# ajbrock/Neural-Photo-Editor

Hardware: NVIDIA H100
Metric: 64x64 images/sec IAN encode->decode @ batch 256 (higher is better)
Workload: dtype f32 (3-pass bf16 split on wgmma, fp32 accumulate)

## Files before the change

### neural-photo-editor_b200/csrc/tapgemm_tc.cu

```cuda
#include <cuda.h>

#include <cstdio>
#include <cstring>
#include <vector>

#include "tapgemm.h"
#include "tc_ptx.cuh"

namespace ian {

struct TcMaps {
  CUtensorMap a[4];
  CUtensorMap b;
  CUtensorMap a1[4];
  CUtensorMap b1;
  CUtensorMap o[2];
  const __nv_bfloat16* o_out;
  long long o_plane;
  int Wt, Ht, Nt, BN;
  mutable int sk_choice;
};

namespace {

using namespace tc;

constexpr int BM = 128;
constexpr int BK = 64;

constexpr int kEpiWarps = 8;
constexpr int kThreadsCta = 32 * kEpiWarps + 32;

template <int BN, int PASSES> struct TcCfg {
  static constexpr int kPlanes = PASSES == 3 ? 2 : 1;
  static constexpr int kATileBytes = BM * BK * 2 * kPlanes;
  static constexpr int kBTileBytes = BN * BK * 2 * kPlanes;
  static constexpr int kStageBytes = kATileBytes + kBTileBytes;
  static constexpr int kRound = (PASSES == 3 && BN > 32) ? 32 : BN;
  static constexpr int kRounds = BN / kRound;
  static constexpr int kLd = kRound + 8;
  static constexpr bool kTmaEpi = PASSES == 3 && BN == 128;
  static constexpr int kOutPlaneBytes = BM * kRound * 2;
  static constexpr int kOutRoundBytes = 2 * kOutPlaneBytes;
  static constexpr int kStagingBytes = kTmaEpi && 2 * kOutRoundBytes > BM * kLd * 4 ? 2 * kOutRoundBytes : BM * kLd * 4;
  static constexpr int kStageSmem = kTmaEpi ? 1024 : kEpiWarps * 1024;
  static constexpr int kStagesFit = (232448 - 1024 - 256 - kStagingBytes - kStageSmem) / kStageBytes;
  static constexpr int kStages = kStagesFit > 6 ? 6 : kStagesFit;
  static constexpr int kSmemBytes = kStages * kStageBytes + 1024  + 256  + kStageSmem + kStagingBytes;
  static_assert(kStages >= 2 && kSmemBytes <= 232448, "tapgemm_tc: shared memory budget");
};
static_assert(TcCfg<128, 3>::kStages == 3 && TcCfg<128, 3>::kSmemBytes == 231680, "tapgemm_tc: three float32-mode stages");
static_assert(TcCfg<128, 3>::kRound == 32 && TcCfg<128, 3>::kOutRoundBytes == 16384, "tapgemm_tc: 32-column TMA-store rounds");

struct WorkItem {
  int phase, ks, co0, it0, it1;
  int n0, p0, q0, mtile;
  int sk_role, sk_last;
};

template <int CH, int PASSES>
__device__ __forceinline__ void store_split(__nv_bfloat16* dst, long long plane, const float (&v)[CH]) {
  __align__(16) __nv_bfloat162 hi[CH / 2], lo[CH / 2];
#pragma unroll
  for (int j = 0; j < CH / 2; ++j) {
    hi[j] = __floats2bfloat162_rn(v[2 * j], v[2 * j + 1]);
    if (PASSES == 3) {
      const float2 hf = __bfloat1622float2(hi[j]);
      lo[j] = __floats2bfloat162_rn(v[2 * j] - hf.x, v[2 * j + 1] - hf.y);
    }
  }
  static_assert(CH % 16 == 0, "an epilogue chunk is a whole number of 32-byte sectors per plane");
  const uint4* h4 = reinterpret_cast<const uint4*>(hi);
  const uint4* l4 = reinterpret_cast<const uint4*>(lo);
#pragma unroll
  for (int j = 0; j < CH / 16; ++j) {
    tc::st_global_256(dst + 16 * j, h4[2 * j], h4[2 * j + 1]);
    if (PASSES == 3) tc::st_global_256(dst + plane + 16 * j, l4[2 * j], l4[2 * j + 1]);
  }
}

template <int BN>
__device__ __forceinline__ WorkItem decode_work(const TapGemm& g, const TcMaps& maps, int w) {
  WorkItem wi;
  const int tiles_q = g.Wg / maps.Wt, tiles_p = g.Hg / maps.Ht;
  const int tiles_m = tiles_q * tiles_p * ((g.n_img + maps.Nt - 1) / maps.Nt);
  const int tiles_n = g.Cout / BN;
  const int per_phase = tiles_m * tiles_n * g.ksplit;
  wi.phase = w / per_phase;
  int r = w % per_phase;
  int mt = r % tiles_m; r /= tiles_m;
  const int nt = r % tiles_n; r /= tiles_n;
  wi.ks = r;
  wi.mtile = mt;
  const int qb = mt % tiles_q; mt /= tiles_q;
  const int pb = mt % tiles_p; mt /= tiles_p;
  wi.n0 = mt * maps.Nt; wi.p0 = pb * maps.Ht; wi.q0 = qb * maps.Wt;
  wi.co0 = nt * BN;
  const int total_it = g.phase[wi.phase].ntaps * (g.Cin / BK);
  wi.it0 = (int)((long long)total_it * wi.ks / g.ksplit);
  wi.it1 = (int)((long long)total_it * (wi.ks + 1) / g.ksplit);
  return wi;
}

template <int BN, bool SK>
struct WorkIter {
  int w, total, stride;
  int T, G, cur, end, iters[kMaxPhases], tiles_per_phase, tiles_m, tiles_q, tiles_p;
  __device__ __forceinline__ int boundary(int c) const { return (int)((long long)T * c / G); }
  __device__ __forceinline__ int owner(int gi) const {
    int c = (int)((long long)gi * G / T);
    while (c + 1 < G && boundary(c + 1) <= gi) ++c;
    while (c > 0 && boundary(c) > gi) --c;
    return c;
  }
  __device__ __forceinline__ void init(const TapGemm& g, const TcMaps& maps, int total_work) {
    if (!SK) { w = blockIdx.x; total = total_work; stride = gridDim.x; return; }
    T = total_work; G = gridDim.x;
    tiles_q = g.Wg / maps.Wt; tiles_p = g.Hg / maps.Ht;
    tiles_m = tiles_q * tiles_p * ((g.n_img + maps.Nt - 1) / maps.Nt);
    tiles_per_phase = tiles_m * (g.Cout / BN);
    for (int p = 0; p < kMaxPhases; ++p) iters[p] = p < g.nphase ? g.phase[p].ntaps * (g.Cin / BK) : 0;
    cur = boundary(blockIdx.x); end = boundary(blockIdx.x + 1);
  }
  __device__ __forceinline__ bool next(const TapGemm& g, const TcMaps& maps, WorkItem& wi) {
    if (!SK) {
      if (w >= total) return false;
      wi = decode_work<BN>(g, maps, w);
      wi.sk_role = 0; wi.sk_last = 0;
      w += stride;
      return true;
    }
    if (cur >= end) return false;
    int gi = cur, ph = 0, phase_start = 0;
    while (ph + 1 < g.nphase && gi >= phase_start + tiles_per_phase * iters[ph]) { phase_start += tiles_per_phase * iters[ph]; ++ph; }
    const int ip = iters[ph];
    const int tile = (gi - phase_start) / ip, it = (gi - phase_start) % ip;
    int len = ip - it;
    if (len > end - gi) len = end - gi;
    wi.phase = ph; wi.ks = 0; wi.it0 = it; wi.it1 = it + len;
    int mt = tile % tiles_m;
    const int nt = tile / tiles_m;
    wi.mtile = mt;
    const int qb = mt % tiles_q; mt /= tiles_q;
    const int pb = mt % tiles_p; mt /= tiles_p;
    wi.n0 = mt * maps.Nt; wi.p0 = pb * maps.Ht; wi.q0 = qb * maps.Wt; wi.co0 = nt * BN;
    wi.sk_role = it > 0 ? 1 : (len < ip ? 2 : 0);
    wi.sk_last = wi.sk_role == 2 ? owner(phase_start + tile * ip + ip - 1) : 0;
    cur = gi + len;
    return true;
  }
};

template <int BN, int PASSES, bool SK>
__global__ void __launch_bounds__(kThreadsCta, 1)
tapgemm_tc_kernel(const __grid_constant__ TapGemm g, const __grid_constant__ TcMaps maps, const int total_work) {
  using Cfg = TcCfg<BN, PASSES>;
  constexpr int kATileBytes = Cfg::kATileBytes;
  constexpr int S = Cfg::kStages;
  extern __shared__ uint8_t smem_raw[];
  const uint32_t smem_base = (smem_u32(smem_raw) + 1023u) & ~1023u;
  const uint32_t stg_base = smem_base + S * Cfg::kStageBytes;
  const uint32_t bar_base = stg_base + Cfg::kStagingBytes;
  auto full_bar = [&](int s) { return bar_base + 8u * s; };
  auto empty_bar = [&](int s) { return bar_base + 8u * (S + s); };
  const uint32_t stage_smem = bar_base + 256u;
  uint8_t* smem_al = smem_raw + (smem_base - smem_u32(smem_raw));
  float* stage_ptr = reinterpret_cast<float*>(smem_al + (stage_smem - smem_base));
  float* acc_tile = reinterpret_cast<float*>(smem_al + (stg_base - smem_base));

  const int warp = threadIdx.x >> 5, lane = threadIdx.x & 31;

  if (threadIdx.x == 0) {
    pdl_trigger();
    for (int s = 0; s < S; ++s) {
      mbar_init(full_bar(s), 1);
      mbar_init(empty_bar(s), 2);
    }
    asm volatile("fence.mbarrier_init.release.cluster;" ::: "memory");
  }
  __syncthreads();
  pdl_wait();

  if (warp == kEpiWarps) {
    uint32_t i = 0;
    WorkIter<BN, SK> iter;
    iter.init(g, maps, total_work);
    WorkItem wi;
    while (iter.next(g, maps, wi)) {
      const Phase ph = g.phase[wi.phase];
      int t = wi.it0 % ph.ntaps, c0 = wi.it0 / ph.ntaps * BK;
      for (int it = wi.it0; it < wi.it1; ++it, ++i) {
        const int s = i % S;
        const uint32_t par = (i / S) & 1u;
        const Tap tap = g.taps[ph.tap_begin + t];
        mbar_wait(empty_bar(s), par ^ 1u);
        const uint32_t sa = smem_base + s * Cfg::kStageBytes;
        if (elect_one_sync()) {
          mbar_expect_tx(full_bar(s), Cfg::kStageBytes);
          tma_load_5d(PASSES == 3 ? &maps.a[tap.view] : &maps.a1[tap.view], full_bar(s), sa, c0, wi.q0 + tap.dw,
                      wi.p0 + tap.dh, wi.n0, 0);
          tma_load_3d(PASSES == 3 ? &maps.b : &maps.b1, full_bar(s), sa + kATileBytes, c0, tap.wtile * g.Cout + wi.co0, 0);
        }
        __syncwarp();
        if (++t == ph.ntaps) { t = 0; c0 += BK; }
      }
    }
    return;
  }

  constexpr int R = BN / 2;
  constexpr int RW = Cfg::kRound;
  constexpr int TC = RW >= 32 ? RW / 2 : RW;
  constexpr int CH = TC >= 32 ? 32 : 16;
  constexpr int kThreadCols = Cfg::kRounds * TC;
  const int wg = warp >> 2, wtid = threadIdx.x & 127;
  const int ew = warp;
  const int lg = warp & 3;
  const int half = ew >> 2;
  const bool has_cols = RW >= 32 || half == 0;
  float* my_stage = stage_ptr + (Cfg::kTmaEpi ? 0 : ew * 256);
  const float act_a = g.act == ACT_LRELU ? 0.6f : g.act == ACT_RELU ? 0.5f : 1.f;
  const float act_b = g.act == ACT_LRELU ? 0.4f : g.act == ACT_RELU ? 0.5f : 0.f;
  const int ml = lg * 32 + lane;
  const int wl0 = ml % maps.Wt;
  const int hl0 = (ml / maps.Wt) % maps.Ht;
  const int nl0 = ml / (maps.Wt * maps.Ht);
  uint32_t i = 0;
  WorkIter<BN, SK> iter;
  iter.init(g, maps, total_work);
  WorkItem wi;
  while (iter.next(g, maps, wi)) {
    const Phase ph = g.phase[wi.phase];
    if (wi.it1 <= wi.it0) continue;
    if (g.scale_pix_stride == 0) {
      if constexpr (Cfg::kTmaEpi) {
        asm volatile("bar.sync 1, 256;" ::: "memory");
        for (int c = threadIdx.x; c < BN; c += 32 * kEpiWarps) {
          my_stage[c] = g.scale ? __ldg(g.scale + wi.co0 + c) : 1.f;
          my_stage[128 + c] = g.shift ? __ldg(g.shift + wi.co0 + c) : 0.f;
        }
      } else if (has_cols) {
        __syncwarp();
        for (int c = lane; c < BN; c += 32) {
          my_stage[c] = g.scale ? __ldg(g.scale + wi.co0 + c) : 1.f;
          my_stage[128 + c] = g.shift ? __ldg(g.shift + wi.co0 + c) : 0.f;
        }
        __syncwarp();
      }
    }
    float acc_m[R], acc_c[PASSES == 3 ? R : 1];
#pragma unroll
    for (int j = 0; j < R; ++j) acc_m[j] = 0.f;
#pragma unroll
    for (int j = 0; j < (PASSES == 3 ? R : 1); ++j) acc_c[j] = 0.f;
    wgmma_fence_regs(acc_m);
    if (PASSES == 3) wgmma_fence_regs(acc_c);
    for (int it = wi.it0; it < wi.it1; ++it, ++i) {
      const int s = i % S;
      mbar_wait(full_bar(s), (i / S) & 1u);
      const uint32_t sa = smem_base + s * Cfg::kStageBytes;
      const uint64_t a_hi = make_sw128_desc(sa + wg * 64 * 128), a_lo = make_sw128_desc(sa + BM * BK * 2 + wg * 64 * 128);
      const uint64_t b_hi = make_sw128_desc(sa + kATileBytes), b_lo = make_sw128_desc(sa + kATileBytes + BN * BK * 2);
      const uint32_t first = (it == wi.it0) ? 0u : 1u;
      wgmma_fence();
#pragma unroll
      for (int k = 0; k < BK / 16; ++k) {
        const uint64_t ko = (uint64_t)(k * 2);
        const uint32_t acc = k > 0 ? 1u : first;
        wgmma_bf16<BN>(acc_m, a_hi + ko, b_hi + ko, acc);
        if constexpr (PASSES == 3) {
          wgmma_bf16<BN>(acc_c, a_lo + ko, b_hi + ko, acc);
          wgmma_bf16<BN>(acc_c, a_hi + ko, b_lo + ko, 1u);
        }
      }
      wgmma_commit();
      wgmma_wait<1>();
      if (it > wi.it0 && wtid == 0) mbar_arrive(empty_bar((i - 1) % S));
    }
    wgmma_wait<0>();
    wgmma_fence_regs(acc_m);
    if (PASSES == 3) wgmma_fence_regs(acc_c);
    if (wtid == 0) mbar_arrive(empty_bar((i - 1) % S));
    if constexpr (PASSES == 3) {
#pragma unroll
      for (int j = 0; j < R; ++j) acc_m[j] += acc_c[j];
    }
    if constexpr (Cfg::kTmaEpi) {
      if (g.epi_tma && wi.sk_role == 0) {
#pragma unroll
        for (int r = 0; r < Cfg::kRounds; ++r) {
          const uint32_t buf = stg_base + (uint32_t)(r & 1) * Cfg::kOutRoundBytes;
          if (threadIdx.x == 0) bulk_wait_group_read1();
          asm volatile("bar.sync 1, 256;" ::: "memory");
#pragma unroll
          for (int j = 0; j < RW / 2; j += 2) {
            const float2 a = make_float2(acc_m[r * RW / 2 + j], acc_m[r * RW / 2 + j + 1]);
            const int row = wg * 64 + frag_row(wtid, j);
            const int c = frag_col(wtid, j);
            const float2 sc = *reinterpret_cast<const float2*>(my_stage + r * RW + c);
            const float2 sf = *reinterpret_cast<const float2*>(my_stage + 128 + r * RW + c);
            float v0 = fmaf(a.x, sc.x, sf.x), v1 = fmaf(a.y, sc.y, sf.y);
            if (g.act == ACT_ELU) {
              v0 = v0 > 0.f ? v0 : expm1f(v0);
              v1 = v1 > 0.f ? v1 : expm1f(v1);
            } else if (g.act != ACT_NONE) {
              v0 = fmaf(act_b, fabsf(v0), act_a * v0);
              v1 = fmaf(act_b, fabsf(v1), act_a * v1);
            }
            const __nv_bfloat162 hi = __floats2bfloat162_rn(v0, v1);
            const float2 hf = __bfloat1622float2(hi);
            const __nv_bfloat162 lo = __floats2bfloat162_rn(v0 - hf.x, v1 - hf.y);
            const uint32_t off = (uint32_t)row * 64u + ((((uint32_t)c >> 3) ^ (((uint32_t)row >> 1) & 3u)) << 4) + ((uint32_t)c & 7u) * 2u;
            asm volatile("st.shared.b32 [%0], %1;" ::"r"(buf + off), "r"(*reinterpret_cast<const uint32_t*>(&hi)) : "memory");
            asm volatile("st.shared.b32 [%0], %1;" ::"r"(buf + Cfg::kOutPlaneBytes + off), "r"(*reinterpret_cast<const uint32_t*>(&lo))
                         : "memory");
          }
          fence_proxy_async_smem();
          asm volatile("bar.sync 1, 256;" ::: "memory");
          if (threadIdx.x == 0) {
            const int c4 = wi.n0 * g.Hg + wi.p0;
            tma_store_5d(&maps.o[0], buf, wi.co0 + r * RW, ph.ow0, wi.q0, ph.oh0, c4);
            tma_store_5d(&maps.o[1], buf + Cfg::kOutPlaneBytes, wi.co0 + r * RW, ph.ow0, wi.q0, ph.oh0, c4);
            bulk_commit_group();
          }
        }
        continue;
      }
      if (threadIdx.x == 0) bulk_wait_group_read0();
    }
    if (SK && wi.sk_role == 2 && has_cols) {
      for (int k = (int)blockIdx.x + 1 + lane; k <= wi.sk_last; k += 32) {
        if (iter.boundary(k) == iter.boundary(k + 1)) continue;
        const int* fl = g.sk_flags + k * kEpiWarps + ew;
        const long long t0 = clock64();
        int fv;
        do {
          asm volatile("ld.acquire.gpu.global.s32 %0, [%1];" : "=r"(fv) : "l"(fl) : "memory");
          if (clock64() - t0 > 4000000000LL) __trap();
        } while (fv != g.sk_epoch);
      }
      __syncwarp();
    }
    int nl = nl0, hl = hl0, wl = wl0;
    if constexpr (SK && Cfg::kTmaEpi) {
      uint32_t tid;
      asm volatile("mov.u32 %0, %%tid.x;" : "=r"(tid));
      const int row = (int)((tid >> 5) & 3u) * 32 + (int)(tid & 31u);
      wl = row % maps.Wt;
      hl = (row / maps.Wt) % maps.Ht;
      nl = row / (maps.Wt * maps.Ht);
    }
    const int n = wi.n0 + nl, p = wi.p0 + hl, q = wi.q0 + wl;
    const bool valid = n < g.n_img;
    const int oh = p * g.osh + ph.oh0, ow = q * g.osw + ph.ow0;
    const long long pix = (long long)(n * g.Hout + oh) * g.Wout + ow;
#pragma unroll 1
    for (int r = 0; r < Cfg::kRounds; ++r) {
      asm volatile("bar.sync 1, 256;" ::: "memory");
#pragma unroll
      for (int j = 0; j < RW / 2; j += 2) {
        float2 v = make_float2(acc_m[j], acc_m[j + 1]);
#pragma unroll
        for (int rr = 1; rr < Cfg::kRounds; ++rr)
          if (rr == r) v = make_float2(acc_m[rr * RW / 2 + j], acc_m[rr * RW / 2 + j + 1]);
        *reinterpret_cast<float2*>(acc_tile + (wg * 64 + frag_row(wtid, j)) * Cfg::kLd + frag_col(wtid, j)) = v;
      }
      asm volatile("bar.sync 1, 256;" ::: "memory");
      if (!has_cols) continue;
#pragma unroll 1
      for (int cc = 0; cc < TC; cc += CH) {
        const int cb = r * RW + half * TC + cc;
        const int co = wi.co0 + cb;
        const int cs = r * TC + cc;
        float v[CH];
        const float* srow = acc_tile + ml * Cfg::kLd + half * TC + cc;
#pragma unroll
        for (int j = 0; j < CH / 4; ++j) {
          const float4 t4 = *reinterpret_cast<const float4*>(srow + 4 * j);
          v[4 * j] = t4.x; v[4 * j + 1] = t4.y; v[4 * j + 2] = t4.z; v[4 * j + 3] = t4.w;
        }
        if (SK && wi.sk_role == 1) {
          float4* wp = reinterpret_cast<float4*>(g.sk_ws + (((long long)blockIdx.x * kEpiWarps + ew) * 32 + lane) * kThreadCols + cs);
#pragma unroll
          for (int j = 0; j < CH / 4; ++j) __stcg(wp + j, make_float4(v[4 * j], v[4 * j + 1], v[4 * j + 2], v[4 * j + 3]));
          continue;
        }
        if (SK && wi.sk_role == 2) {
          for (int k = (int)blockIdx.x + 1; k <= wi.sk_last; ++k) {
            if (iter.boundary(k) == iter.boundary(k + 1)) continue;
            const float4* rp = reinterpret_cast<const float4*>(g.sk_ws + (((long long)k * kEpiWarps + ew) * 32 + lane) * kThreadCols + cs);
#pragma unroll
            for (int j = 0; j < CH / 4; ++j) {
              const float4 a = __ldcg(rp + j);
              v[4 * j] += a.x; v[4 * j + 1] += a.y; v[4 * j + 2] += a.z; v[4 * j + 3] += a.w;
            }
          }
        }
        if (g.ksplit > 1) {
          if (valid) {
            float4* wsp = reinterpret_cast<float4*>(g.ws + (long long)wi.ks * g.ws_slab + pix * g.Cout + co);
#pragma unroll
            for (int j = 0; j < CH / 4; ++j) __stcg(wsp + j, make_float4(v[4 * j], v[4 * j + 1], v[4 * j + 2], v[4 * j + 3]));
          }
          continue;
        }
        if (valid) {
          const long long off = pix * g.Cout + co;
          if (g.out_raw) store_split<CH, PASSES>(g.out_raw + off, g.out_raw_plane, v);
          if (g.res && !g.res_after) {
            const uint4* rh = reinterpret_cast<const uint4*>(g.res + off);
            const uint4* rl = reinterpret_cast<const uint4*>(g.res + g.res_plane + off);
#pragma unroll
            for (int j8 = 0; j8 < CH / 8; ++j8) {
              const uint4 h4 = __ldg(rh + j8);
              const __nv_bfloat16* hb = reinterpret_cast<const __nv_bfloat16*>(&h4);
              if (PASSES == 3) {
                const uint4 l4 = __ldg(rl + j8);
                const __nv_bfloat16* lb = reinterpret_cast<const __nv_bfloat16*>(&l4);
#pragma unroll
                for (int j = 0; j < 8; ++j) v[j8 * 8 + j] += __bfloat162float(hb[j]) + __bfloat162float(lb[j]);
              } else {
#pragma unroll
                for (int j = 0; j < 8; ++j) v[j8 * 8 + j] += __bfloat162float(hb[j]);
              }
            }
          }
          if (g.act == ACT_MASK) {
            const int si = co + (oh * g.Wout + ow) * g.scale_pix_stride;
            const uint4* mk = reinterpret_cast<const uint4*>(g.mask + off);
#pragma unroll
            for (int j8 = 0; j8 < CH / 8; ++j8) {
              const uint4 m4 = __ldg(mk + j8);
              const __nv_bfloat16* mb = reinterpret_cast<const __nv_bfloat16*>(&m4);
#pragma unroll
              for (int j = 0; j < 8; ++j) {
                const float sc = g.scale_pix_stride ? __ldg(g.scale + si + j8 * 8 + j) : my_stage[cb + j8 * 8 + j];
                v[j8 * 8 + j] = v[j8 * 8 + j] * sc * (__bfloat162float(mb[j]) > 0.f ? 1.f : g.mask_slope);
              }
            }
            if (g.res && g.res_after) {
              const uint4* rh = reinterpret_cast<const uint4*>(g.res + off);
              const uint4* rl = reinterpret_cast<const uint4*>(g.res + g.res_plane + off);
#pragma unroll
              for (int j8 = 0; j8 < CH / 8; ++j8) {
                const uint4 h4 = __ldg(rh + j8);
                const __nv_bfloat16* hb = reinterpret_cast<const __nv_bfloat16*>(&h4);
                if (PASSES == 3) {
                  const uint4 l4 = __ldg(rl + j8);
                  const __nv_bfloat16* lb = reinterpret_cast<const __nv_bfloat16*>(&l4);
#pragma unroll
                  for (int j = 0; j < 8; ++j) v[j8 * 8 + j] += __bfloat162float(hb[j]) + __bfloat162float(lb[j]);
                } else {
#pragma unroll
                  for (int j = 0; j < 8; ++j) v[j8 * 8 + j] += __bfloat162float(hb[j]);
                }
              }
            }
          } else {
#pragma unroll
            for (int j4 = 0; j4 < CH / 4; ++j4) {
              const float4 sc = *reinterpret_cast<const float4*>(my_stage + cb + 4 * j4);
              const float4 sf = *reinterpret_cast<const float4*>(my_stage + 128 + cb + 4 * j4);
              v[4 * j4 + 0] = fmaf(v[4 * j4 + 0], sc.x, sf.x);
              v[4 * j4 + 1] = fmaf(v[4 * j4 + 1], sc.y, sf.y);
              v[4 * j4 + 2] = fmaf(v[4 * j4 + 2], sc.z, sf.z);
              v[4 * j4 + 3] = fmaf(v[4 * j4 + 3], sc.w, sf.w);
            }
            if (g.act == ACT_ELU) {
#pragma unroll
              for (int j = 0; j < CH; ++j) v[j] = v[j] > 0.f ? v[j] : expm1f(v[j]);
            } else if (g.act != ACT_NONE) {
#pragma unroll
              for (int j = 0; j < CH; ++j) v[j] = fmaf(act_b, fabsf(v[j]), act_a * v[j]);
            }
          }
          if (g.out) store_split<CH, PASSES>(g.out + off, g.out_plane, v);
          if (g.out_f32_t) {
            const long long tbase = ((long long)wi.mtile * g.cout_real + co) * BM + ml;
            if (g.out_t_bf16) {
              __nv_bfloat16* ot = reinterpret_cast<__nv_bfloat16*>(g.out_f32_t) + tbase;
#pragma unroll
              for (int j = 0; j < CH; ++j)
                if (co + j < g.cout_real) ot[j * BM] = __float2bfloat16_rn(v[j]);
            } else {
              float* ot = g.out_f32_t + tbase;
#pragma unroll
              for (int j = 0; j < CH; ++j)
                if (co + j < g.cout_real) ot[j * BM] = v[j];
            }
          }
          if (g.out_f32) {
            float4* of = reinterpret_cast<float4*>(g.out_f32 + off);
#pragma unroll
            for (int j = 0; j < CH / 4; ++j) of[j] = make_float4(v[4 * j], v[4 * j + 1], v[4 * j + 2], v[4 * j + 3]);
          }
        }
      }
    }
    if (SK && wi.sk_role == 1 && has_cols) {
      __threadfence();
      __syncwarp();
      if (lane == 0) {
        int* fl = g.sk_flags + (int)blockIdx.x * kEpiWarps + ew;
        asm volatile("st.release.gpu.global.s32 [%0], %1;" ::"l"(fl), "r"(g.sk_epoch) : "memory");
      }
    }
  }
  if constexpr (Cfg::kTmaEpi) {
    if (threadIdx.x == 0) bulk_wait_group0();
  }
}

}

TcMaps* tc_build_maps(const TapGemm& g, char* err, int errlen) {
  tc::EncodeTiledFn enc = tc::get_encode_fn();
  if (!enc) { snprintf(err, errlen, "cuTensorMapEncodeTiled entry point not available"); return nullptr; }
  if (g.Cin % 64 || (g.Cout % 128 && g.Cout != 16)) { snprintf(err, errlen, "tc path needs Cin%%64==0 and Cout%%128==0 or Cout==16 (got %d,%d)", g.Cin, g.Cout); return nullptr; }
  TcMaps* m = new TcMaps();
  memset(m, 0, sizeof(*m));
  tile_shape(g.Hg, g.Wg, m->Wt, m->Ht, m->Nt);
  m->sk_choice = -1;
  m->BN = (g.Cout % 128 == 0) ? 128 : 16;
  if (g.Wg % m->Wt || g.Hg % m->Ht || m->Wt * m->Ht * m->Nt != BM) {
    snprintf(err, errlen, "M grid %dx%d does not tile into 128-row boxes", g.Hg, g.Wg);
    delete m; return nullptr;
  }
  bool used[4] = {false, false, false, false};
  int max_tile = 0;
  for (int p = 0; p < g.nphase; ++p)
    for (int t = 0; t < g.phase[p].ntaps; ++t) {
      const Tap& tp = g.taps[g.phase[p].tap_begin + t];
      used[tp.view] = true;
      if (tp.wtile > max_tile) max_tile = tp.wtile;
    }
  for (int v = 0; v < 4; ++v) {
    if (!used[v]) continue;
    const int vh = v >> 1, vw = v & 1;
    const cuuint64_t Hv = (g.Hin - vh + g.sh - 1) / g.sh, Wv = (g.Win - vw + g.sw - 1) / g.sw;
    cuuint64_t dims[5] = {(cuuint64_t)g.Cin, Wv, Hv, (cuuint64_t)g.n_img, 2};
    cuuint64_t strides[4] = {(cuuint64_t)g.sw * g.Cin * 2, (cuuint64_t)g.sh * g.Win * g.Cin * 2,
                             (cuuint64_t)g.Hin * g.Win * g.Cin * 2, (cuuint64_t)g.a_plane * 2};
    cuuint32_t box[5] = {BK, (cuuint32_t)m->Wt, (cuuint32_t)m->Ht, (cuuint32_t)m->Nt, 2};
    cuuint32_t estr[5] = {1, 1, 1, 1, 1};
    void* base = (void*)(g.a + ((long long)vh * g.Win + vw) * g.Cin);
    CUresult r = enc(&m->a[v], CU_TENSOR_MAP_DATA_TYPE_BFLOAT16, 5, base, dims, strides, box, estr,
                     CU_TENSOR_MAP_INTERLEAVE_NONE, CU_TENSOR_MAP_SWIZZLE_128B, CU_TENSOR_MAP_L2_PROMOTION_L2_256B,
                     CU_TENSOR_MAP_FLOAT_OOB_FILL_NONE);
    if (r != CUDA_SUCCESS) { snprintf(err, errlen, "cuTensorMapEncodeTiled(A view %d) failed: %d", v, (int)r); delete m; return nullptr; }
    box[4] = 1;
    r = enc(&m->a1[v], CU_TENSOR_MAP_DATA_TYPE_BFLOAT16, 5, base, dims, strides, box, estr, CU_TENSOR_MAP_INTERLEAVE_NONE,
            CU_TENSOR_MAP_SWIZZLE_128B, CU_TENSOR_MAP_L2_PROMOTION_L2_256B, CU_TENSOR_MAP_FLOAT_OOB_FILL_NONE);
    if (r != CUDA_SUCCESS) { snprintf(err, errlen, "cuTensorMapEncodeTiled(A1 view %d) failed: %d", v, (int)r); delete m; return nullptr; }
  }
  {
    cuuint64_t dims[3] = {(cuuint64_t)g.Cin, (cuuint64_t)(max_tile + 1) * g.Cout, 2};
    cuuint64_t strides[2] = {(cuuint64_t)g.Cin * 2, (cuuint64_t)g.b_plane * 2};
    cuuint32_t box[3] = {BK, (cuuint32_t)m->BN, 2};
    cuuint32_t estr[3] = {1, 1, 1};
    CUresult r = enc(&m->b, CU_TENSOR_MAP_DATA_TYPE_BFLOAT16, 3, (void*)g.b, dims, strides, box, estr,
                     CU_TENSOR_MAP_INTERLEAVE_NONE, CU_TENSOR_MAP_SWIZZLE_128B, CU_TENSOR_MAP_L2_PROMOTION_L2_256B,
                     CU_TENSOR_MAP_FLOAT_OOB_FILL_NONE);
    if (r != CUDA_SUCCESS) { snprintf(err, errlen, "cuTensorMapEncodeTiled(B) failed: %d", (int)r); delete m; return nullptr; }
    box[2] = 1;
    r = enc(&m->b1, CU_TENSOR_MAP_DATA_TYPE_BFLOAT16, 3, (void*)g.b, dims, strides, box, estr, CU_TENSOR_MAP_INTERLEAVE_NONE,
            CU_TENSOR_MAP_SWIZZLE_128B, CU_TENSOR_MAP_L2_PROMOTION_L2_256B, CU_TENSOR_MAP_FLOAT_OOB_FILL_NONE);
    if (r != CUDA_SUCCESS) { snprintf(err, errlen, "cuTensorMapEncodeTiled(B1) failed: %d", (int)r); delete m; return nullptr; }
  }
  if (g.out && m->BN == 128 && g.Hout == g.osh * g.Hg && g.Wout == g.osw * g.Wg && (g.out_plane * 2) % 16 == 0 &&
      (uintptr_t)g.out % 16 == 0) {
    const cuuint64_t C = (cuuint64_t)g.Cout;
    cuuint64_t dims[5] = {C, (cuuint64_t)g.osw, (cuuint64_t)g.Wg, (cuuint64_t)g.osh, (cuuint64_t)g.n_img * g.Hg};
    cuuint64_t strides[4] = {C * 2, C * 2 * g.osw, C * 2 * g.Wout, C * 2 * g.Wout * g.osh};
    cuuint32_t box[5] = {32, 1, (cuuint32_t)m->Wt, 1, (cuuint32_t)(m->Ht * m->Nt)};
    cuuint32_t estr[5] = {1, 1, 1, 1, 1};
    bool ok = true;
    for (int pl = 0; pl < 2 && ok; ++pl)
      ok = enc(&m->o[pl], CU_TENSOR_MAP_DATA_TYPE_BFLOAT16, 5, (void*)(g.out + pl * g.out_plane), dims, strides, box, estr,
               CU_TENSOR_MAP_INTERLEAVE_NONE, CU_TENSOR_MAP_SWIZZLE_64B, CU_TENSOR_MAP_L2_PROMOTION_NONE,
               CU_TENSOR_MAP_FLOAT_OOB_FILL_NONE) == CUDA_SUCCESS;
    if (ok) { m->o_out = g.out; m->o_plane = g.out_plane; }
  }
  return m;
}

void tc_free_maps(TcMaps* m) { delete m; }

int tc_tile_width(const TcMaps* maps) { return maps->BN; }

int tc_num_sms() {
  static std::atomic<int> num_sms[kMaxDevices];
  const int dev = cur_device();
  int n = num_sms[dev].load(std::memory_order_relaxed);
  if (!n) {
    cudaDeviceGetAttribute(&n, cudaDevAttrMultiProcessorCount, dev);
    num_sms[dev].store(n, std::memory_order_relaxed);
  }
  return n;
}
size_t tc_sk_workspace_floats() { return (size_t)tc_num_sms() * kEpiWarps * 32 * 128; }
size_t tc_sk_flag_ints() { return (size_t)tc_num_sms() * kEpiWarps; }

template <int BN, int PASSES, bool SK>
static int launch_one(const TapGemm& g, const TcMaps* maps, int tiles_m, int num_sms, cudaStream_t st) {
  using Cfg = TcCfg<BN, PASSES>;
  static DeviceOnce attr_set;
  const int dev = cur_device();
  if (!attr_set.is_done(dev)) {
    if (cudaFuncSetAttribute(tapgemm_tc_kernel<BN, PASSES, SK>, cudaFuncAttributeMaxDynamicSharedMemorySize, Cfg::kSmemBytes) != cudaSuccess)
      return -1;
    attr_set.set_done(dev);
  }
  int total_work, grid;
  if (SK) {
    long long T = 0;
    for (int p = 0; p < g.nphase; ++p) T += (long long)tiles_m * (g.Cout / maps->BN) * g.phase[p].ntaps * (g.Cin / BK);
    total_work = (int)T;
    grid = num_sms;
  } else {
    total_work = tiles_m * (g.Cout / maps->BN) * g.nphase * g.ksplit;
    grid = total_work < num_sms ? total_work : num_sms;
  }
  if (launch_pdl(tapgemm_tc_kernel<BN, PASSES, SK>, dim3(grid), dim3(kThreadsCta), Cfg::kSmemBytes, st, g, *maps, total_work) != cudaSuccess)
    return -1;
  return cudaGetLastError() == cudaSuccess ? 1 : -1;
}

int launch_tapgemm_tc(const TapGemm& g_in, const TcMaps* maps, cudaStream_t st) {
  TapGemm g = g_in;
  g.epi_tma = g_in.epi_tma && g.passes == 3 && maps->BN == 128 && g.ksplit == 1 && g.out && g.out == maps->o_out &&
              g.out_plane == maps->o_plane && g.scale_pix_stride == 0 &&
              (g.act == ACT_NONE || g.act == ACT_LRELU || g.act == ACT_RELU || g.act == ACT_ELU) && !g.out_raw && !g.res &&
              !g.mask && !g.out_f32 && !g.out_f32_t;
  const int num_sms = tc_num_sms();
  const int tiles_m = (g.Wg / maps->Wt) * (g.Hg / maps->Ht) * ((g.n_img + maps->Nt - 1) / maps->Nt);
  const long long tiles = (long long)tiles_m * (g.Cout / maps->BN) * g.nphase;
  bool sk = false;
  if (g.sk_force) {
    sk = g.sk_ws && g.ksplit == 1 && maps->BN == 128 && !g.out_f32_t;
  } else if (maps->sk_choice >= 0) {
    sk = maps->sk_choice == 1 && g.sk_ws != nullptr;
  } else if (g.sk_ws && g.ksplit == 1 && maps->BN == 128 && tiles >= num_sms / 2 && !g.out_f32_t) {
    const int per_phase = tiles_m * (g.Cout / maps->BN);
    std::vector<long long> load(num_sms, 0);
    long long T = 0;
    for (long long w = 0; w < tiles; ++w) {
      const int it = g.phase[w / per_phase].ntaps * (g.Cin / BK);
      load[w % num_sms] += it;
      T += it;
    }
    long long makespan = 0;
    for (long long v : load) makespan = v > makespan ? v : makespan;
    sk = makespan * num_sms >= (T * 6) / 5;
    maps->sk_choice = sk ? 1 : 0;
  } else if (g.sk_ws) {
    maps->sk_choice = 0;
  }
  if (g.passes == 1) {
    if (maps->BN == 128) return sk ? launch_one<128, 1, true>(g, maps, tiles_m, num_sms, st) : launch_one<128, 1, false>(g, maps, tiles_m, num_sms, st);
    return launch_one<16, 1, false>(g, maps, tiles_m, num_sms, st);
  }
  if (maps->BN == 128) return sk ? launch_one<128, 3, true>(g, maps, tiles_m, num_sms, st) : launch_one<128, 3, false>(g, maps, tiles_m, num_sms, st);
  return launch_one<16, 3, false>(g, maps, tiles_m, num_sms, st);
}

}
```

### neural-photo-editor_b200/csrc/tc_ptx.cuh

```cuda
#pragma once
#include <cuda.h>
#include <stdint.h>

namespace ian {
namespace tc {

__device__ __forceinline__ uint32_t smem_u32(const void* p) { return (uint32_t)__cvta_generic_to_shared(p); }

__device__ __forceinline__ bool elect_one_sync() {
  uint32_t pred;
  asm volatile(
      "{\n\t.reg .pred P1;\n\t"
      "elect.sync _|P1, 0xffffffff;\n\t"
      "selp.b32 %0, 1, 0, P1;\n\t}"
      : "=r"(pred));
  return pred != 0;
}

__device__ __forceinline__ void st_global_256(void* p, const uint4& a, const uint4& b) {
  asm volatile("st.global.v4.b32 [%0], {%1, %2, %3, %4};" ::"l"(p), "r"(a.x), "r"(a.y), "r"(a.z), "r"(a.w) : "memory");
  asm volatile("st.global.v4.b32 [%0], {%1, %2, %3, %4};" ::"l"(reinterpret_cast<uint8_t*>(p) + 16), "r"(b.x), "r"(b.y),
               "r"(b.z), "r"(b.w)
               : "memory");
}

__device__ __forceinline__ void mbar_init(uint32_t bar, uint32_t count) {
  asm volatile("mbarrier.init.shared::cta.b64 [%0], %1;" ::"r"(bar), "r"(count) : "memory");
}
__device__ __forceinline__ void mbar_expect_tx(uint32_t bar, uint32_t bytes) {
  asm volatile("mbarrier.arrive.expect_tx.shared::cta.b64 _, [%0], %1;" ::"r"(bar), "r"(bytes) : "memory");
}
__device__ __forceinline__ void mbar_arrive(uint32_t bar) {
  asm volatile("mbarrier.arrive.shared::cta.b64 _, [%0];" ::"r"(bar) : "memory");
}
__device__ __forceinline__ bool mbar_try_wait(uint32_t bar, uint32_t parity) {
  uint32_t ok;
  asm volatile(
      "{\n\t.reg .pred p;\n\t"
      "mbarrier.try_wait.parity.shared::cta.b64 p, [%1], %2;\n\t"
      "selp.u32 %0, 1, 0, p;\n\t}"
      : "=r"(ok)
      : "r"(bar), "r"(parity)
      : "memory");
  return ok != 0;
}
__device__ __forceinline__ void mbar_wait(uint32_t bar, uint32_t parity) {
  if (mbar_try_wait(bar, parity)) return;
  const long long t0 = clock64();
  while (!mbar_try_wait(bar, parity)) {
    if (clock64() - t0 > 4000000000LL) __trap();
  }
}

__device__ __forceinline__ void tma_load_5d(const CUtensorMap* map, uint32_t bar, uint32_t dst, int c0, int c1, int c2,
                                            int c3, int c4) {
  asm volatile(
      "cp.async.bulk.tensor.5d.shared::cluster.global.mbarrier::complete_tx::bytes [%0], [%1, {%3, %4, %5, %6, %7}], [%2];"
      ::"r"(dst), "l"(map), "r"(bar), "r"(c0), "r"(c1), "r"(c2), "r"(c3), "r"(c4)
      : "memory");
}
__device__ __forceinline__ void tma_load_3d(const CUtensorMap* map, uint32_t bar, uint32_t dst, int c0, int c1, int c2) {
  asm volatile(
      "cp.async.bulk.tensor.3d.shared::cluster.global.mbarrier::complete_tx::bytes [%0], [%1, {%3, %4, %5}], [%2];"
      ::"r"(dst), "l"(map), "r"(bar), "r"(c0), "r"(c1), "r"(c2)
      : "memory");
}

__device__ __forceinline__ void tma_store_3d(const CUtensorMap* map, uint32_t src, int c0, int c1, int c2) {
  asm volatile("cp.async.bulk.tensor.3d.global.shared::cta.bulk_group [%0, {%2, %3, %4}], [%1];" ::"l"(map), "r"(src), "r"(c0),
               "r"(c1), "r"(c2)
               : "memory");
}
__device__ __forceinline__ void tma_store_5d(const CUtensorMap* map, uint32_t src, int c0, int c1, int c2, int c3, int c4) {
  asm volatile("cp.async.bulk.tensor.5d.global.shared::cta.bulk_group [%0, {%2, %3, %4, %5, %6}], [%1];" ::"l"(map), "r"(src),
               "r"(c0), "r"(c1), "r"(c2), "r"(c3), "r"(c4)
               : "memory");
}
__device__ __forceinline__ void bulk_commit_group() { asm volatile("cp.async.bulk.commit_group;" ::: "memory"); }
__device__ __forceinline__ void bulk_wait_group_read0() { asm volatile("cp.async.bulk.wait_group.read 0;" ::: "memory"); }
__device__ __forceinline__ void bulk_wait_group_read1() { asm volatile("cp.async.bulk.wait_group.read 1;" ::: "memory"); }
__device__ __forceinline__ void bulk_wait_group0() { asm volatile("cp.async.bulk.wait_group 0;" ::: "memory"); }
__device__ __forceinline__ void fence_proxy_async_smem() { asm volatile("fence.proxy.async.shared::cta;" ::: "memory"); }
__device__ __forceinline__ void st_shared_v4(uint32_t addr, const uint4& v) {
  asm volatile("st.shared.v4.b32 [%0], {%1, %2, %3, %4};" ::"r"(addr), "r"(v.x), "r"(v.y), "r"(v.z), "r"(v.w) : "memory");
}

__device__ __forceinline__ void wgmma_fence() { asm volatile("wgmma.fence.sync.aligned;" ::: "memory"); }
__device__ __forceinline__ void wgmma_commit() { asm volatile("wgmma.commit_group.sync.aligned;" ::: "memory"); }
template <int N> __device__ __forceinline__ void wgmma_wait() { asm volatile("wgmma.wait_group.sync.aligned %0;" ::"n"(N) : "memory"); }
template <int R> __device__ __forceinline__ void wgmma_fence_regs(float (&d)[R]) {
#pragma unroll
  for (int j = 0; j < R; ++j) asm volatile("" : "+f"(d[j])::"memory");
}

template <int N> __device__ __forceinline__ void wgmma_bf16(float (&d)[N / 2], uint64_t a, uint64_t b, uint32_t accum);
template <> __device__ __forceinline__ void wgmma_bf16<16>(float (&d)[8], uint64_t a, uint64_t b, uint32_t accum) {
  asm volatile(
      "{\n\t.reg .pred p;\n\t"
      "setp.ne.b32 p, %10, 0;\n\t"
      "wgmma.mma_async.sync.aligned.m64n16k16.f32.bf16.bf16 "
      "{%0, %1, %2, %3, %4, %5, %6, %7}, %8, %9, p, 1, 1, 0, 0;\n\t}"
      : "+f"(d[0]), "+f"(d[1]), "+f"(d[2]), "+f"(d[3]), "+f"(d[4]), "+f"(d[5]), "+f"(d[6]), "+f"(d[7])
      : "l"(a), "l"(b), "r"(accum));
}
template <> __device__ __forceinline__ void wgmma_bf16<40>(float (&d)[20], uint64_t a, uint64_t b, uint32_t accum) {
  asm volatile(
      "{\n\t.reg .pred p;\n\t"
      "setp.ne.b32 p, %22, 0;\n\t"
      "wgmma.mma_async.sync.aligned.m64n40k16.f32.bf16.bf16 "
      "{%0, %1, %2, %3, %4, %5, %6, %7, %8, %9, %10, %11, %12, %13, %14, %15, %16, %17, %18, %19}, %20, %21, p, 1, 1, 0, 0;\n\t}"
      : "+f"(d[0]), "+f"(d[1]), "+f"(d[2]), "+f"(d[3]), "+f"(d[4]), "+f"(d[5]), "+f"(d[6]), "+f"(d[7]), "+f"(d[8]), "+f"(d[9]), "+f"(d[10]), "+f"(d[11]), "+f"(d[12]), "+f"(d[13]), "+f"(d[14]), "+f"(d[15]), "+f"(d[16]), "+f"(d[17]), "+f"(d[18]), "+f"(d[19])
      : "l"(a), "l"(b), "r"(accum));
}
template <> __device__ __forceinline__ void wgmma_bf16<64>(float (&d)[32], uint64_t a, uint64_t b, uint32_t accum) {
  asm volatile(
      "{\n\t.reg .pred p;\n\t"
      "setp.ne.b32 p, %34, 0;\n\t"
      "wgmma.mma_async.sync.aligned.m64n64k16.f32.bf16.bf16 "
      "{%0, %1, %2, %3, %4, %5, %6, %7, %8, %9, %10, %11, %12, %13, %14, %15, %16, %17, %18, %19, %20, %21, %22, %23, %24, %25, %26, %27, %28, %29, %30, %31}, %32, %33, p, 1, 1, 0, 0;\n\t}"
      : "+f"(d[0]), "+f"(d[1]), "+f"(d[2]), "+f"(d[3]), "+f"(d[4]), "+f"(d[5]), "+f"(d[6]), "+f"(d[7]), "+f"(d[8]), "+f"(d[9]), "+f"(d[10]), "+f"(d[11]), "+f"(d[12]), "+f"(d[13]), "+f"(d[14]), "+f"(d[15]), "+f"(d[16]), "+f"(d[17]), "+f"(d[18]), "+f"(d[19]), "+f"(d[20]), "+f"(d[21]), "+f"(d[22]), "+f"(d[23]), "+f"(d[24]), "+f"(d[25]), "+f"(d[26]), "+f"(d[27]), "+f"(d[28]), "+f"(d[29]), "+f"(d[30]), "+f"(d[31])
      : "l"(a), "l"(b), "r"(accum));
}
template <> __device__ __forceinline__ void wgmma_bf16<80>(float (&d)[40], uint64_t a, uint64_t b, uint32_t accum) {
  asm volatile(
      "{\n\t.reg .pred p;\n\t"
      "setp.ne.b32 p, %42, 0;\n\t"
      "wgmma.mma_async.sync.aligned.m64n80k16.f32.bf16.bf16 "
      "{%0, %1, %2, %3, %4, %5, %6, %7, %8, %9, %10, %11, %12, %13, %14, %15, %16, %17, %18, %19, %20, %21, %22, %23, %24, %25, %26, %27, %28, %29, %30, %31, %32, %33, %34, %35, %36, %37, %38, %39}, %40, %41, p, 1, 1, 0, 0;\n\t}"
      : "+f"(d[0]), "+f"(d[1]), "+f"(d[2]), "+f"(d[3]), "+f"(d[4]), "+f"(d[5]), "+f"(d[6]), "+f"(d[7]), "+f"(d[8]), "+f"(d[9]), "+f"(d[10]), "+f"(d[11]), "+f"(d[12]), "+f"(d[13]), "+f"(d[14]), "+f"(d[15]), "+f"(d[16]), "+f"(d[17]), "+f"(d[18]), "+f"(d[19]), "+f"(d[20]), "+f"(d[21]), "+f"(d[22]), "+f"(d[23]), "+f"(d[24]), "+f"(d[25]), "+f"(d[26]), "+f"(d[27]), "+f"(d[28]), "+f"(d[29]), "+f"(d[30]), "+f"(d[31]), "+f"(d[32]), "+f"(d[33]), "+f"(d[34]), "+f"(d[35]), "+f"(d[36]), "+f"(d[37]), "+f"(d[38]), "+f"(d[39])
      : "l"(a), "l"(b), "r"(accum));
}
template <> __device__ __forceinline__ void wgmma_bf16<128>(float (&d)[64], uint64_t a, uint64_t b, uint32_t accum) {
  asm volatile(
      "{\n\t.reg .pred p;\n\t"
      "setp.ne.b32 p, %66, 0;\n\t"
      "wgmma.mma_async.sync.aligned.m64n128k16.f32.bf16.bf16 "
      "{%0, %1, %2, %3, %4, %5, %6, %7, %8, %9, %10, %11, %12, %13, %14, %15, %16, %17, %18, %19, %20, %21, %22, %23, %24, %25, %26, %27, %28, %29, %30, %31, %32, %33, %34, %35, %36, %37, %38, %39, %40, %41, %42, %43, %44, %45, %46, %47, %48, %49, %50, %51, %52, %53, %54, %55, %56, %57, %58, %59, %60, %61, %62, %63}, %64, %65, p, 1, 1, 0, 0;\n\t}"
      : "+f"(d[0]), "+f"(d[1]), "+f"(d[2]), "+f"(d[3]), "+f"(d[4]), "+f"(d[5]), "+f"(d[6]), "+f"(d[7]), "+f"(d[8]), "+f"(d[9]), "+f"(d[10]), "+f"(d[11]), "+f"(d[12]), "+f"(d[13]), "+f"(d[14]), "+f"(d[15]), "+f"(d[16]), "+f"(d[17]), "+f"(d[18]), "+f"(d[19]), "+f"(d[20]), "+f"(d[21]), "+f"(d[22]), "+f"(d[23]), "+f"(d[24]), "+f"(d[25]), "+f"(d[26]), "+f"(d[27]), "+f"(d[28]), "+f"(d[29]), "+f"(d[30]), "+f"(d[31]), "+f"(d[32]), "+f"(d[33]), "+f"(d[34]), "+f"(d[35]), "+f"(d[36]), "+f"(d[37]), "+f"(d[38]), "+f"(d[39]), "+f"(d[40]), "+f"(d[41]), "+f"(d[42]), "+f"(d[43]), "+f"(d[44]), "+f"(d[45]), "+f"(d[46]), "+f"(d[47]), "+f"(d[48]), "+f"(d[49]), "+f"(d[50]), "+f"(d[51]), "+f"(d[52]), "+f"(d[53]), "+f"(d[54]), "+f"(d[55]), "+f"(d[56]), "+f"(d[57]), "+f"(d[58]), "+f"(d[59]), "+f"(d[60]), "+f"(d[61]), "+f"(d[62]), "+f"(d[63])
      : "l"(a), "l"(b), "r"(accum));
}

template <int N> __device__ __forceinline__ void wgmma_bf16_mn(float (&d)[N / 2], uint64_t a, uint64_t b, uint32_t accum);
template <> __device__ __forceinline__ void wgmma_bf16_mn<128>(float (&d)[64], uint64_t a, uint64_t b, uint32_t accum) {
  asm volatile(
      "{\n\t.reg .pred p;\n\t"
      "setp.ne.b32 p, %66, 0;\n\t"
      "wgmma.mma_async.sync.aligned.m64n128k16.f32.bf16.bf16 "
      "{%0, %1, %2, %3, %4, %5, %6, %7, %8, %9, %10, %11, %12, %13, %14, %15, %16, %17, %18, %19, %20, %21, %22, %23, %24, %25, %26, %27, %28, %29, %30, %31, %32, %33, %34, %35, %36, %37, %38, %39, %40, %41, %42, %43, %44, %45, %46, %47, %48, %49, %50, %51, %52, %53, %54, %55, %56, %57, %58, %59, %60, %61, %62, %63}, %64, %65, p, 1, 1, 1, 1;\n\t}"
      : "+f"(d[0]), "+f"(d[1]), "+f"(d[2]), "+f"(d[3]), "+f"(d[4]), "+f"(d[5]), "+f"(d[6]), "+f"(d[7]), "+f"(d[8]), "+f"(d[9]), "+f"(d[10]), "+f"(d[11]), "+f"(d[12]), "+f"(d[13]), "+f"(d[14]), "+f"(d[15]), "+f"(d[16]), "+f"(d[17]), "+f"(d[18]), "+f"(d[19]), "+f"(d[20]), "+f"(d[21]), "+f"(d[22]), "+f"(d[23]), "+f"(d[24]), "+f"(d[25]), "+f"(d[26]), "+f"(d[27]), "+f"(d[28]), "+f"(d[29]), "+f"(d[30]), "+f"(d[31]), "+f"(d[32]), "+f"(d[33]), "+f"(d[34]), "+f"(d[35]), "+f"(d[36]), "+f"(d[37]), "+f"(d[38]), "+f"(d[39]), "+f"(d[40]), "+f"(d[41]), "+f"(d[42]), "+f"(d[43]), "+f"(d[44]), "+f"(d[45]), "+f"(d[46]), "+f"(d[47]), "+f"(d[48]), "+f"(d[49]), "+f"(d[50]), "+f"(d[51]), "+f"(d[52]), "+f"(d[53]), "+f"(d[54]), "+f"(d[55]), "+f"(d[56]), "+f"(d[57]), "+f"(d[58]), "+f"(d[59]), "+f"(d[60]), "+f"(d[61]), "+f"(d[62]), "+f"(d[63])
      : "l"(a), "l"(b), "r"(accum));
}

__device__ __forceinline__ int frag_row(int tid, int j) { return 16 * (tid >> 5) + ((tid & 31) >> 2) + 8 * ((j >> 1) & 1); }
__device__ __forceinline__ int frag_col(int tid, int j) { return 8 * (j >> 2) + 2 * (tid & 3) + (j & 1); }

__device__ __forceinline__ uint64_t make_sw128_desc(uint32_t saddr) {
  uint64_t d = 0;
  d |= (uint64_t)((saddr & 0x3FFFF) >> 4);
  d |= (uint64_t)1 << 16;
  d |= (uint64_t)(1024 >> 4) << 32;
  d |= (uint64_t)1 << 62;
  return d;
}

__device__ __forceinline__ uint64_t make_sw128_mn_desc(uint32_t saddr, uint32_t lbo_bytes) {
  uint64_t d = 0;
  d |= (uint64_t)((saddr & 0x3FFFF) >> 4);
  d |= (uint64_t)((lbo_bytes >> 4) & 0x3FFF) << 16;
  d |= (uint64_t)(1024 >> 4) << 32;
  d |= (uint64_t)1 << 62;
  return d;
}

typedef CUresult (*EncodeTiledFn)(CUtensorMap*, CUtensorMapDataType, cuuint32_t, void*, const cuuint64_t*,
                                  const cuuint64_t*, const cuuint32_t*, const cuuint32_t*, CUtensorMapInterleave,
                                  CUtensorMapSwizzle, CUtensorMapL2promotion, CUtensorMapFloatOOBfill);

inline EncodeTiledFn get_encode_fn() {
  static EncodeTiledFn fn = nullptr;
  if (!fn) {
    void* p = nullptr;
    cudaDriverEntryPointQueryResult qres;
    if (cudaGetDriverEntryPoint("cuTensorMapEncodeTiled", &p, cudaEnableDefault, &qres) != cudaSuccess ||
        qres != cudaDriverEntryPointSuccess)
      return nullptr;
    fn = reinterpret_cast<EncodeTiledFn>(p);
  }
  return fn;
}

}
}
```

Measured before the change: 86460.

## Split 3-pass wgmma into two commit groups and async-load epilogue scale/shift

The 3-pass loop now issues the correction products (lo*hi, hi*lo) as one commit group, waits for the previous group, releases the prior stage, then issues the main hi*hi products as a second group. The aim is to release smem stages earlier and keep more wgmma work in flight. In the TMA-epilogue path, per-channel scale/shift are fetched with cp.async (one element per thread) instead of a barrier plus a load loop, so the fetch overlaps the mainloop. A barrier at the end of each work item plus cp.async waits replace the old barrier. This assumes BN<=128 and 256 epilogue threads, and the extra wait and barrier points could add stalls.

```diff
diff --git a/neural-photo-editor_b200/csrc/tapgemm_tc.cu b/neural-photo-editor_b200/csrc/tapgemm_tc.cu
--- a/neural-photo-editor_b200/csrc/tapgemm_tc.cu
+++ b/neural-photo-editor_b200/csrc/tapgemm_tc.cu
@@ -234,11 +234,10 @@
     if (wi.it1 <= wi.it0) continue;
     if (g.scale_pix_stride == 0) {
       if constexpr (Cfg::kTmaEpi) {
-        asm volatile("bar.sync 1, 256;" ::: "memory");
-        for (int c = threadIdx.x; c < BN; c += 32 * kEpiWarps) {
-          my_stage[c] = g.scale ? __ldg(g.scale + wi.co0 + c) : 1.f;
-          my_stage[128 + c] = g.shift ? __ldg(g.shift + wi.co0 + c) : 0.f;
-        }
+        const float* src = threadIdx.x < 128 ? g.scale : g.shift;
+        float* dst = my_stage + threadIdx.x;
+        if (src) cp_async_4(smem_u32(dst), src + wi.co0 + (threadIdx.x & 127));
+        else *dst = threadIdx.x < 128 ? 1.f : 0.f;
       } else if (has_cols) {
         __syncwarp();
         for (int c = lane; c < BN; c += 32) {
@@ -263,19 +262,32 @@
       const uint64_t b_hi = make_sw128_desc(sa + kATileBytes), b_lo = make_sw128_desc(sa + kATileBytes + BN * BK * 2);
       const uint32_t first = (it == wi.it0) ? 0u : 1u;
       wgmma_fence();
-#pragma unroll
-      for (int k = 0; k < BK / 16; ++k) {
-        const uint64_t ko = (uint64_t)(k * 2);
-        const uint32_t acc = k > 0 ? 1u : first;
-        wgmma_bf16<BN>(acc_m, a_hi + ko, b_hi + ko, acc);
-        if constexpr (PASSES == 3) {
-          wgmma_bf16<BN>(acc_c, a_lo + ko, b_hi + ko, acc);
+      if constexpr (PASSES == 3) {
+#pragma unroll
+        for (int k = 0; k < BK / 16; ++k) {
+          const uint64_t ko = (uint64_t)(k * 2);
+          wgmma_bf16<BN>(acc_c, a_lo + ko, b_hi + ko, k > 0 ? 1u : first);
           wgmma_bf16<BN>(acc_c, a_hi + ko, b_lo + ko, 1u);
         }
-      }
-      wgmma_commit();
-      wgmma_wait<1>();
-      if (it > wi.it0 && wtid == 0) mbar_arrive(empty_bar((i - 1) % S));
+        wgmma_commit();
+        wgmma_wait<1>();
+        if (it > wi.it0 && wtid == 0) mbar_arrive(empty_bar((i - 1) % S));
+#pragma unroll
+        for (int k = 0; k < BK / 16; ++k) {
+          const uint64_t ko = (uint64_t)(k * 2);
+          wgmma_bf16<BN>(acc_m, a_hi + ko, b_hi + ko, k > 0 ? 1u : first);
+        }
+        wgmma_commit();
+      } else {
+#pragma unroll
+        for (int k = 0; k < BK / 16; ++k) {
+          const uint64_t ko = (uint64_t)(k * 2);
+          wgmma_bf16<BN>(acc_m, a_hi + ko, b_hi + ko, k > 0 ? 1u : first);
+        }
+        wgmma_commit();
+        wgmma_wait<1>();
+        if (it > wi.it0 && wtid == 0) mbar_arrive(empty_bar((i - 1) % S));
+      }
     }
     wgmma_wait<0>();
     wgmma_fence_regs(acc_m);
@@ -290,6 +302,7 @@
 #pragma unroll
         for (int r = 0; r < Cfg::kRounds; ++r) {
           const uint32_t buf = stg_base + (uint32_t)(r & 1) * Cfg::kOutRoundBytes;
+          if (r == 0) cp_async_wait_all();
           if (threadIdx.x == 0) bulk_wait_group_read1();
           asm volatile("bar.sync 1, 256;" ::: "memory");
 #pragma unroll
@@ -327,6 +340,7 @@
         continue;
       }
       if (threadIdx.x == 0) bulk_wait_group_read0();
+      cp_async_wait_all();
     }
     if (SK && wi.sk_role == 2 && has_cols) {
       for (int k = (int)blockIdx.x + 1 + lane; k <= wi.sk_last; k += 32) {
@@ -505,6 +519,7 @@
         asm volatile("st.release.gpu.global.s32 [%0], %1;" ::"l"(fl), "r"(g.sk_epoch) : "memory");
       }
     }
+    if constexpr (Cfg::kTmaEpi) asm volatile("bar.sync 1, 256;" ::: "memory");
   }
   if constexpr (Cfg::kTmaEpi) {
     if (threadIdx.x == 0) bulk_wait_group0();
diff --git a/neural-photo-editor_b200/csrc/tc_ptx.cuh b/neural-photo-editor_b200/csrc/tc_ptx.cuh
--- a/neural-photo-editor_b200/csrc/tc_ptx.cuh
+++ b/neural-photo-editor_b200/csrc/tc_ptx.cuh
@@ -81,6 +81,10 @@
 __device__ __forceinline__ void bulk_wait_group_read1() { asm volatile("cp.async.bulk.wait_group.read 1;" ::: "memory"); }
 __device__ __forceinline__ void bulk_wait_group0() { asm volatile("cp.async.bulk.wait_group 0;" ::: "memory"); }
 __device__ __forceinline__ void fence_proxy_async_smem() { asm volatile("fence.proxy.async.shared::cta;" ::: "memory"); }
+__device__ __forceinline__ void cp_async_4(uint32_t dst, const float* src) {
+  asm volatile("cp.async.ca.shared.global [%0], [%1], 4;" ::"r"(dst), "l"(src) : "memory");
+}
+__device__ __forceinline__ void cp_async_wait_all() { asm volatile("cp.async.wait_all;" ::: "memory"); }
 __device__ __forceinline__ void st_shared_v4(uint32_t addr, const uint4& v) {
   asm volatile("st.shared.v4.b32 [%0], {%1, %2, %3, %4};" ::"r"(addr), "r"(v.x), "r"(v.y), "r"(v.z), "r"(v.w) : "memory");
 }
```

Result: faster. 88530, median of 6 (+2.4%).
